# Aakash1312/Fluid-Simulation

Measured on AMD Instinct MI355X. Metric: simulated substeps/sec, higher is better.
Workload: dtype f64

## Files before the change

fluid-simulation_amd/csrc/common.h:

```cpp
#pragma once
#include <hip/hip_runtime.h>
#include <stdint.h>

namespace fl {

constexpr uint8_t F_SOLID = 1;
constexpr uint8_t F_FLUID = 2;
constexpr int F_CNT_SHIFT = 2;

struct Grid {
    int N;
    int lo;
    int hi;
    int nx, ny, nz;
    int ox, oy, oz;
    __host__ __device__ inline size_t idx(int ix, int iy, int iz) const
    {
        return ((size_t)ix * ny + (size_t)iy) * nz + (size_t)iz;
    }
    __host__ __device__ inline size_t cells() const { return (size_t)nx * ny * nz; }
    __host__ __device__ inline long sx() const { return (long)ny * nz; }
    __host__ __device__ inline int cx0() const { return lo + ox; }
    __host__ __device__ inline int cy0() const { return lo + oy; }
    __host__ __device__ inline int cz0() const { return lo + oz; }
    __host__ __device__ inline int cx1() const { return lo + ox + nx - 1; }
    __host__ __device__ inline int cy1() const { return lo + oy + ny - 1; }
    __host__ __device__ inline int cz1() const { return lo + oz + nz - 1; }
};

struct Box {
    int x0, y0, z0, x1, y1, z1;
    __host__ __device__ inline int nx() const { return x1 - x0 + 1; }
    __host__ __device__ inline int ny() const { return y1 - y0 + 1; }
    __host__ __device__ inline int nz() const { return z1 - z0 + 1; }
    __host__ __device__ inline long long cells() const { return (long long)nx() * ny() * nz(); }
};

template <typename T>
struct Coef {
    T diag[7];
    T inv[7];
    T off;
};

constexpr int LBOX_K0 = 16;
struct LBox {
    int x0, y0, z0, nx, ny, nz, Lx, Ly, Lz;
    __host__ __device__ inline size_t cells() const { return (size_t)Lx * Ly * Lz; }
};

struct MLevel {
    int dx, dy, dz;
    long sx, sy;
    int ox, oy, oz;
    size_t cells;
    __host__ __device__ inline size_t at(int i, int j, int k) const
    {
        return (size_t)((long)(i + ox) * sx + (long)(j + oy) * sy + (k + oz));
    }
};
template <typename T>
struct MgCoef {
    T diag[7];
    T inv[7];
    T off;
};

struct PcgState {
    double bb;
    double thr;
    double rr;
    int done;
    int iters;
    int breakdown;
    int pad;
};

struct StepState {
    int bbox_min[3];
    int bbox_max[3];
    int num_active;
    int n_out;
    int max_cell;
    int n_drop;
    int n_tl_mg, n_tl_sq;
    int n_rows, n_l1_old;
    int n_tl_int, n_tl_bnd;
    int n_l1_gal, n_drop_fail;
    unsigned long long max_speed_bits;
    double dt;
    double err_num;
    double err_den;
};

constexpr size_t STATE_PS_OFF = 256;
constexpr int MAX_PARTIALS = 8192;

__device__ __forceinline__ double spline(double x)
{
    if (x < 0) x *= -1.0;
    if (x < 0.5) return 1.5 * (4.0 * x * x * x - 4.0 * x * x + 2.0 / 3.0);
    if (x < 1.0) return 1.5 * ((-8.0 * (x * x * x) / 6.0) + 4.0 * x * x - 4.0 * x + 4.0 / 3.0);
    return 0;
}

__device__ __forceinline__ double spline_at(double p, int c, int d)
{
    double x = p - (double)c;
    if (d == 1) return spline(x);
    if (x < 0) x *= -1.0;
    if (x < 1.0) return 1.5 * ((-8.0 * (x * x * x) / 6.0) + 4.0 * x * x - 4.0 * x + 4.0 / 3.0);
    return 0;
}

template <typename T>
__device__ __forceinline__ T wave_sum(T v)
{
#pragma unroll
    for (int o = 32; o > 0; o >>= 1) v += __shfl_down(v, o, 64);
    return v;
}
template <typename T>
__device__ __forceinline__ T wave_max(T v)
{
#pragma unroll
    for (int o = 32; o > 0; o >>= 1) {
        T w = __shfl_down(v, o, 64);
        v = w > v ? w : v;
    }
    return v;
}
template <typename T, int NW>
__device__ __forceinline__ T block_sum(T v, T* sm)
{
    v = wave_sum(v);
    const int lane = threadIdx.x & 63, w = threadIdx.x >> 6;
    __syncthreads();
    if (lane == 0) sm[w] = v;
    __syncthreads();
    T r = 0;
    if (threadIdx.x == 0) {
#pragma unroll
        for (int i = 0; i < NW; ++i) r += sm[i];
    }
    return r;
}
template <int NW>
__device__ __forceinline__ double block_sum_array(const double* __restrict__ a, int n, double* sm)
{
    double v = 0;
    for (int i = threadIdx.x; i < n; i += NW * 64) v += a[i];
    v = wave_sum(v);
    const int lane = threadIdx.x & 63, w = threadIdx.x >> 6;
    __syncthreads();
    if (lane == 0) sm[w] = v;
    __syncthreads();
    if (threadIdx.x == 0) {
        double r = 0;
#pragma unroll
        for (int i = 0; i < NW; ++i) r += sm[i];
        sm[NW] = r;
    }
    __syncthreads();
    return sm[NW];
// ... 136 lines not shown
void launch_pcg_sq_list(hipStream_t st, LBox L, const uint8_t* cnt, const T* r, const T* s_in, T* s_out, T* q, Coef<T> cf,
                        const double* part_rr, int n_prev, const double* part_rz_new, const double* part_rz_old, double* part_pq, PcgState* ps,
                        int first, double tol, int n_rz, int zmode, const int* tlist, int nlist);
template <typename T>
void launch_pcg_xr_list(hipStream_t st, LBox L, const uint8_t* cnt, T* x, T* r, const T* s, const T* q, Coef<T> cf, const double* part_rz_cur,
                        int n_rz, const double* part_pq, double* part_rr, double* part_rz_next, PcgState* ps, const int* tlist, int nlist);
int pcg_row_count(const LBox& L);
int pcg_rows_blocks(int nrows);
void launch_row_list(hipStream_t st, LBox L, const uint8_t* cnt, int* flags, int* pos, int* list, int* block_sums, int* count);
constexpr int DROP_CAP = 65536;
constexpr int DROP_NCTR = 64;
void launch_drop_find(hipStream_t st, LBox L, uint8_t* cnt, int* ctr, int* pre, int* total, int* comp_n, int* comp_cells, const Box* own = nullptr);
void launch_drop_solve(hipStream_t st, Grid g, LBox L, int n_comp, const int* pre, const int* comp_n, const int* comp_cells, const uint8_t* flags,
                       const float* b, Coef<double> cf, double tol, double* pressure, double* keep, int* n_fail = nullptr, const PcgState* gate = nullptr);
template <typename T>
void launch_pcg_xr_rows(hipStream_t st, LBox L, const uint8_t* cnt, T* x, T* r, const T* s, const T* q, Coef<T> cf, const double* part_rz_cur,
                        int n_rz, const double* part_pq, int n_pq, double* part_rr, double* part_rz_next, PcgState* ps, const int* rlist, int nrows);
template <typename T>
void launch_pcg_sq_dist(hipStream_t st, LBox L, const uint8_t* cnt, const T* r, const T* s_in, T* s_out, T* q, Coef<T> cf, const double* g_rr,
                        const double* g_rz_new, const double* g_rz_old, double* part_pq, PcgState* ps, int first, double tol, int zmode);
template <typename T>
void launch_pcg_xr_dist(hipStream_t st, LBox L, const uint8_t* cnt, T* x, T* r, const T* s, const T* q, Coef<T> cf, const double* g_rz_cur,
                        const double* g_pq, double* part_rr, double* part_rz_next, PcgState* ps);
void launch_sum2(hipStream_t st, const double* a, int na, const double* b, int nb, double* out_a, double* out_b);
void launch_pcg_az_dist_zf(hipStream_t st, LBox L, const uint8_t* cnt, const float* z, double* w, Coef<double> cf, double* part_zw, PcgState* ps, const int* tlist, int nlist);
void launch_pcg_cgear_upd_zf(hipStream_t st, LBox L, const uint8_t* cnt, double* x, double* r, double* s, double* q, const float* z, const double* w, const double* g,
                             double* cg, int cur, double* part_rr, PcgState* ps, int first, double tol);
void launch_pcg_poll_stage(hipStream_t st, const double* part_rr, int n, const PcgState* ps, double* out);
void launch_pcg_poll_test(hipStream_t st, const double* g, PcgState* ps);
void launch_sum4(hipStream_t st, const double* a, int na, const double* b, int nb, const double* c, int nc, const double* e, int ne, double* out);
template <typename T>
void launch_pcg_az_dist(hipStream_t st, LBox L, const uint8_t* cnt, const T* z, T* w, Coef<T> cf, double* part_zw, PcgState* ps, const int* tlist = nullptr,
                        int nlist = 0);
template <typename T>
void launch_pcg_cgear_upd(hipStream_t st, LBox L, const uint8_t* cnt, T* x, T* r, T* s, T* q, const T* z, const T* w, const double* g, double* cg, int cur,
                          double* part_rr, PcgState* ps, int first, double tol);
template <typename T>
void launch_stencil_apply(hipStream_t st, Grid g, Box box, const uint8_t* flags, const T* s, T* q, Coef<T> cf);
template <typename T>
bool launch_stencil_march(hipStream_t st, Grid g, const uint8_t* flags, const T* s, T* q, Coef<T> cf, int variant, int cxcode);
template <typename T>
void launch_store_pressure(hipStream_t st, Grid g, LBox L, const uint8_t* cnt, const T* x, double* pressure, double* keep = nullptr,
                           const PcgState* ps = nullptr, bool gated = false);
template <typename T>
void launch_pcg_init_guess(hipStream_t st, Grid g, LBox L, const uint8_t* cnt, const float* b, const double* guess, const double* guess2, double ca,
                           double cb, T* x, T* r, Coef<T> cf, double* part_bb, double* part_rr0, PcgState* ps);

MLevel mg_level0(const LBox& L);
MLevel mg_coarser(const MLevel& f);
void launch_mg_type0(hipStream_t st, Grid g, LBox L, MLevel m, const uint8_t* flags, const uint8_t* cnt, uint8_t* typ);
void launch_mg_coarsen(hipStream_t st, MLevel mf, const uint8_t* tf, MLevel mc, uint8_t* tc, uint8_t* cnt_c);
void launch_mg_coarsen_types(hipStream_t st, MLevel mf, const uint8_t* tf, MLevel mc, uint8_t* tc);
void launch_mg_counts(hipStream_t st, MLevel m, const uint8_t* typ, uint8_t* cnt);
template <typename T>
void launch_mg_restrict(hipStream_t st, MLevel mf, const T* rf, MLevel mc, const uint8_t* cnt_c, T* fc, const PcgState* ps);
constexpr int MG_TAIL_MAX = 4;
constexpr size_t MG_TAIL_LDS = 144 * 1024;
size_t mg_tail_lds_bytes(int nl, const MLevel* lv, size_t elem);
int mg_up_blocks(const MLevel& m);
template <typename T, typename F>
void launch_mg_down(hipStream_t st, MLevel m, const uint8_t* cnt, const F* f, T* u, T* r, MLevel mc, const uint8_t* cnt_c, T* fc, MgCoef<T> cf,
                    const PcgState* ps, const int* tlist = nullptr, int nlist = 0, bool pcr = false);
template <typename T, typename F, typename O>
void launch_mg_up(hipStream_t st, MLevel m, const uint8_t* cnt, const F* f, const T* u, O* out, MLevel mc, const T* ec, MgCoef<T> cf,
                  double* part_dot, const PcgState* ps, double wc, const int* tlist = nullptr, int nlist = 0, const uint8_t* own = nullptr,
                  int pconst = 0);
bool gal_fits_coarsest(const MLevel& m);
void launch_gal_level1(hipStream_t st, MLevel m0, const uint8_t* cnt0, MgCoef<float> cf0, MLevel m1, float* gd, float* gx, float* gy, float* gz, uint8_t* cnt1);
void launch_gal_coarsen(hipStream_t st, MLevel mf, const float* fd, const float* fx, const float* fy, const float* fz, const uint8_t* cntf, MLevel mc,
                        float* gd, float* gx, float* gy, float* gz, uint8_t* cntc);
int gal_tile_count(const MLevel& m);
void launch_gal_tile_flags(hipStream_t st, MLevel m, const uint8_t* cnt, uint8_t* flags);
void launch_gal_down(hipStream_t st, MLevel m, const uint8_t* cnt, const float* gd, const float* gx, const float* gy, const float* gz, const float* f, float* u,
                     MLevel mc, float* fc, const PcgState* ps);
void launch_gal_up(hipStream_t st, MLevel m, const uint8_t* cnt, const float* gd, const float* gx, const float* gy, const float* gz, const float* f, const float* u,
                   float* out, MLevel mc, const float* ec, float wc, const PcgState* ps);
void launch_gal_coarsest(hipStream_t st, MLevel m, const float* gd, const float* gx, const float* gy, const float* gz, const float* f, float* u, int sweeps,
                         const PcgState* ps);
void launch_mg_tile_flags(hipStream_t st, MLevel m, const uint8_t* cnt, uint8_t* flags);
void launch_sq_tile_flags(hipStream_t st, LBox L, const uint8_t* cnt, uint8_t* flags);
int sq_tile_count(const LBox& L);
void launch_compact_flags(hipStream_t st, const uint8_t* flags, int n, int* list, int* count);
template <typename T>
void launch_mg_tail(hipStream_t st, int nl, const T* f0, const MLevel* lv, uint8_t* const* cnt, T* u0, const T* off, int sweeps, const PcgState* ps,
                    double wc);

}
```

fluid-simulation_amd/csrc/fluid_api.hip:

```cpp
#include "sim.h"
#include <algorithm>

using namespace fl;

static thread_local std::string g_err;
int fluid_fail(int code, const std::string& msg)
{
    g_err = msg;
    return code;
}
#define fail fluid_fail

Box fl::clip_dilate(const Box& b, int d, const Grid& g)
{
    Box r;
    r.x0 = b.x0 - d < 0 ? 0 : b.x0 - d;
    r.y0 = b.y0 - d < 0 ? 0 : b.y0 - d;
    r.z0 = b.z0 - d < 0 ? 0 : b.z0 - d;
    r.x1 = b.x1 + d > g.nx - 1 ? g.nx - 1 : b.x1 + d;
    r.y1 = b.y1 + d > g.ny - 1 ? g.ny - 1 : b.y1 + d;
    r.z1 = b.z1 + d > g.nz - 1 ? g.nz - 1 : b.z1 + d;
    return r;
}

// ... 151 lines not shown
    if (s->h_ss) hipHostFree(s->h_ss);
    if (s->h_small) hipHostFree(s->h_small);
    if (s->st) hipStreamDestroy(s->st);
    delete s;
    return FLUID_OK;
}

int fluid_create(const fluid_params_t* p, fluid_sim_t** out)
{
    if (!p || !out) return fail(FLUID_ERR_ARG, "null argument");
    Grid g;
    g.N = p->n;
    g.lo = -(p->n / 2);
    g.hi = g.lo + p->n - 1;
    g.nx = g.ny = g.nz = p->n;
    g.ox = g.oy = g.oz = 0;
    return fluid_create_window(p, g, out);
}

}

int fl::fluid_create_window(const fluid_params_t* p, const Grid& g, fluid_sim_t** out)
{
    if (!p || !out) return fail(FLUID_ERR_ARG, "null argument");
    if (p->n < 8 || p->n > 1024) return fail(FLUID_ERR_ARG, "n must be in [8,1024]");
    if (!(p->dx > 0) || !(p->rho > 0) || !(p->max_dt > 0)) return fail(FLUID_ERR_ARG, "dx, rho, max_dt must be > 0");
    if (p->precision != FLUID_PRECISION_FP64 && p->precision != FLUID_PRECISION_FP32) return fail(FLUID_ERR_ARG, "bad precision");
    if (!(p->flip_blend >= 0.0 && p->flip_blend <= 1.0)) return fail(FLUID_ERR_ARG, "flip_blend must be in [0,1] (1 = the reference's pure FLIP)");
    if (p->preconditioner != FLUID_PRECOND_MG && p->preconditioner != FLUID_PRECOND_JACOBI) return fail(FLUID_ERR_ARG, "bad preconditioner");
    if (p->solve_start != FLUID_START_WARM && p->solve_start != FLUID_START_ZERO) return fail(FLUID_ERR_ARG, "bad solve_start");
    if (p->mg_precision != FLUID_MG_FP32 && p->mg_precision != FLUID_MG_FP64) return fail(FLUID_ERR_ARG, "bad mg_precision");
    if (p->dist_solve < FLUID_DIST_AUTO || p->dist_solve > FLUID_DIST_REPLICATED || p->pad_ != 0) return fail(FLUID_ERR_ARG, "bad dist_solve / pad_");
    int ndev = 0;
    if (hipGetDeviceCount(&ndev) != hipSuccess || ndev <= 0)
        return fail(FLUID_ERR_HIP, "no HIP device visible: libfluid_hip has no CPU path");
    if (p->device < 0 || p->device >= ndev) return fail(FLUID_ERR_ARG, "device ordinal out of range");
    HIPCHK(hipSetDevice(p->device));
    fluid_sim* s = new fluid_sim();
    s->prm = *p;
    s->g = g;
    s->ncell = g.cells();
    s->dt = p->max_dt;
    s->mg_fp32 = p->mg_precision == FLUID_MG_FP32;
    s->warm = p->solve_start == FLUID_START_WARM;
    if (const char* e = getenv("FLUID_MG_CSWEEPS")) s->mg_csweeps = atoi(e);
    if (const char* e = getenv("FLUID_TILE_LISTS")) s->lists_force = atoi(e) != 0;
    if (const char* e = getenv("FLUID_P2G_FORM")) s->p2g_force = !strcmp(e, "rows") ? 1 : (!strcmp(e, "tiles") ? 2 : (!strcmp(e, "crowd") ? 3 : 0));
    if (const char* e = getenv("FLUID_MG_GALERKIN")) s->gal_mode = atoi(e);
    if (const char* e = getenv("FLUID_DROPLETS")) s->drops_on = atoi(e) != 0;
    if (const char* e = getenv("FLUID_ROW_SWEEPS")) s->row_sweeps = atoi(e) != 0;
    if (const char* e = getenv("FLUID_DROPLETS_MIN")) s->drop_min = atoi(e);
    if (const char* e = getenv("FLUID_ADVECT_BIN")) s->advect_bin = atoi(e) != 0;
    if (const char* e = getenv("FLUID_SOLVE_TAIL")) s->solve_tail = atoi(e) != 0;
    *out = nullptr;
    auto bail = [&](int rc) { fluid_destroy(s); return rc; };
#define A(expr) do { hipError_t e_ = (expr); if (e_ != hipSuccess) return bail(fail(FLUID_ERR_HIP, std::string(#expr) + ": " + hipGetErrorString(e_))); } while (0)
    A(hipStreamCreateWithFlags(&s->st, hipStreamNonBlocking));
    const size_t n = s->ncell;
    A(dalloc(&s->solid, n)); A(dalloc(&s->flags, n));
    A(dalloc(&s->container, n)); A(dalloc(&s->rhs, n)); A(dalloc(&s->diver, n)); A(dalloc(&s->diver2, n));
    A(dalloc(&s->u, n)); A(dalloc(&s->v, n)); A(dalloc(&s->w, n));
    A(dalloc(&s->ub, n)); A(dalloc(&s->vb, n)); A(dalloc(&s->wb, n));
    A(dalloc(&s->dcx, n)); A(dalloc(&s->dcy, n)); A(dalloc(&s->dcz, n));
    A(dalloc(&s->pressure, n));
    if (s->warm) {
        A(dalloc(&s->p_guess, n)); A(dalloc(&s->p_guess2, n));
        if (hipMemset(s->p_guess, 0, n * sizeof(double)) != hipSuccess || hipMemset(s->p_guess2, 0, n * sizeof(double)) != hipSuccess) return bail(FLUID_ERR_HIP);
        if (const char* e = getenv("FLUID_EXTRAPOLATE")) s->extrapolate = atoi(e) != 0;
        if (s->extrapolate) { A(dalloc(&s->p_q, n)); if (hipMemset(s->p_q, 0, n * sizeof(double)) != hipSuccess) return bail(FLUID_ERR_HIP); }
    }
    A(dalloc(&s->indices, n));
    A(dalloc(&s->scan_sums, (n + 2) / 2048 + 16));
    A(dalloc(&s->ipart, (size_t)1024 * 8));
    const size_t se = solver_elem(s);
    s->lmax = lbox_max_cells(std::max(g.nx, std::max(g.ny, g.nz)));
    const size_t ln = s->lmax;
    A(dalloc((char**)&s->R, ln * se)); A(dalloc((char**)&s->S[0], 2 * ln * se + 256));
    s->S[1] = (char*)s->S[0] + ln * se;
    A(dalloc((char**)&s->Q, ln * se)); A(dalloc((char**)&s->X, ln * se)); A(dalloc(&s->cntL, ln + 64));
    A(dalloc(&s->mg_part, ln / 256 + 64));
    A(dalloc(&s->part_bb, (size_t)MAX_PARTIALS)); A(dalloc(&s->part_rr, (size_t)MAX_PARTIALS));
    A(dalloc(&s->part_rz[0], (size_t)MAX_PARTIALS)); A(dalloc(&s->part_rz[1], (size_t)MAX_PARTIALS));
    A(dalloc(&s->part_pq, (size_t)MAX_PARTIALS)); A(dalloc(&s->part_err, (size_t)2 * MAX_PARTIALS));
    static_assert(sizeof(StepState) <= STATE_PS_OFF, "PcgState overlaps StepState");
    A(dalloc((char**)&s->ss, STATE_PS_OFF + sizeof(PcgState)));
    s->ps = (PcgState*)((char*)s->ss + STATE_PS_OFF);
    A(dalloc(&s->cell_count, n + 4)); A(dalloc(&s->cell_start, n + 4));
    A(dalloc(&s->d_small, (size_t)32));
    A(hipHostMalloc((void**)&s->h_small, 32 * sizeof(int)));
    A(hipEventCreateWithFlags(&s->ev_poll[0], hipEventDisableTiming));
    A(hipEventCreateWithFlags(&s->ev_poll[1], hipEventDisableTiming));
    A(hipHostMalloc((void**)&s->h_ss, STATE_PS_OFF + 2 * sizeof(PcgState)));
    s->h_ps = (PcgState*)((char*)s->h_ss + STATE_PS_OFF);
#undef A
    std::vector<uint8_t> sol(n, 0);
    const int N = p->n;
    for (int x = 0; x < g.nx; ++x)
        for (int y = 0; y < g.ny; ++y)
            for (int z = 0; z < g.nz; ++z) {
                const int X = x + g.ox, Y = y + g.oy, Z = z + g.oz;
                if (X < 2 || X > N - 3 || Y < 2 || Y > N - 3 || Z < 2 || Z > N - 3) sol[g.idx(x, y, z)] = 1;
            }
    hipError_t e = hipMemcpy(s->solid, sol.data(), n, hipMemcpyHostToDevice);
    if (e == hipSuccess) e = hipMemcpy(s->flags, sol.data(), n, hipMemcpyHostToDevice);
    if (e == hipSuccess) e = hipDeviceSynchronize();
    if (e != hipSuccess) return bail(fail(FLUID_ERR_HIP, std::string("solid upload: ") + hipGetErrorString(e)));
// ... 263 lines not shown
    int rc = phase_sort(s);
    if (rc) return rc;
    rc = clear_dirty(s);
    if (rc) return rc;
    memset(&s->stats, 0, sizeof(s->stats));
    s->stats.dt_in = s->dt;
    s->stats.dt_out = s->dt;
    for (int a = 0; a < 3; ++a) {
        s->stats.box_lo[a] = (&s->Rb.x0)[a];
        s->stats.box_hi[a] = (&s->Rb.x1)[a];
    }
    if (!box_empty(s->Rb)) {
        int tok = prof_begin(s, FLUID_PROF_P2G, (double)s->Rb.cells());
        rc = run_p2g(s, s->Rb);
        prof_end(s, FLUID_PROF_P2G, tok);
        if (rc) return rc;
        HIPCHK(hipGetLastError());
        s->dirty = s->Sb;
    }
    s->have_p2g = true;
    s->step_counter++;
    s->have_flags = false;
    return FLUID_OK;
}

template <typename T>
Coef<T> fl::make_coef(const fluid_sim* s)
{
    const double scale = s->dt / (s->prm.rho * s->prm.dx * s->prm.dx);
    Coef<T> c;
    float acc = 0.0f;
    c.diag[0] = 0;
    c.inv[0] = 0;
    for (int k = 1; k <= 6; ++k) {
        acc = (float)((double)acc + scale);
        c.diag[k] = (T)acc;
        c.inv[k] = (T)1 / c.diag[k];
    }
    c.off = (T)(float)(-1 * scale);
    return c;
}
template Coef<double> fl::make_coef<double>(const fluid_sim*);
template Coef<float> fl::make_coef<float>(const fluid_sim*);

hipError_t fl::zero_search(fluid_sim* s, size_t lb)
{
    const size_t step = (lb + 255) / 256 * 256;
    s->S[1] = (char*)s->S[0] + step;
    return hipMemsetAsync(s->S[0], 0, step + lb, s->st);
}


static int gal_build(fluid_sim* s);
static int mg_setup(fluid_sim* s)
{
    s->mgl[0] = mg_level0(s->L);
    int nl = 1;
    while (nl < fluid_sim::MG_MAXL && (nl < 2 || s->mgl[nl - 1].dx > 8 || s->mgl[nl - 1].dy > 8 || s->mgl[nl - 1].dz > 8)) {
        s->mgl[nl] = mg_coarser(s->mgl[nl - 1]);
        ++nl;
    }
    if (s->mgl[nl - 1].dx > 8 || s->mgl[nl - 1].dy > 8 || s->mgl[nl - 1].dz > 8) return fail(FLUID_ERR_STATE, "multigrid: too many levels");
    s->mg_nl = nl;
    int tail = nl - 1;
    const size_t es = s->mg_fp32 ? sizeof(float) : sizeof(double);
    auto fits = [&](int t) {
        const size_t b = nl - t <= MG_TAIL_MAX ? mg_tail_lds_bytes(nl - t, s->mgl + t, es) : 0;
        return b > 0 && b <= MG_TAIL_LDS;
    };
    while (tail > 1 && fits(tail - 1)) --tail;
    if (!fits(tail)) return fail(FLUID_ERR_STATE, "multigrid: coarsest level does not fit the tail kernel");
    s->mg_tail = tail;
    size_t total = 0;
    auto take = [&](size_t bytes) { const size_t o = total; total += (bytes + 255) / 256 * 256; return o; };
    size_t o_typ[fluid_sim::MG_MAXL], o_cnt[fluid_sim::MG_MAXL], o_u[fluid_sim::MG_MAXL], o_v[fluid_sim::MG_MAXL], o_f[fluid_sim::MG_MAXL],
        o_r[fluid_sim::MG_MAXL];
    for (int l = 0; l < nl; ++l) {
        const size_t c = s->mgl[l].cells + 64;
        o_typ[l] = take(c); o_cnt[l] = take(c);
        o_u[l] = take(c * es); o_v[l] = take(c * es); o_f[l] = take(c * es); o_r[l] = take(c * es);
    }
    const size_t o_z = take((s->mgl[0].cells + 64) * 8);
    if (total > s->mg_slab_cap) {
        if (s->mg_slab) { HIPCHK(hipStreamSynchronize(s->st)); hipFree(s->mg_slab); s->mg_slab = nullptr; }
        const size_t cap = total + total / 4;
        HIPCHK(hipMalloc((void**)&s->mg_slab, cap));
        s->mg_slab_cap = cap;
    }
    for (int l = 0; l < nl; ++l) {
        s->mg_typ[l] = (uint8_t*)(s->mg_slab + o_typ[l]);
        s->mg_cnt[l] = l ? (uint8_t*)(s->mg_slab + o_cnt[l]) : nullptr;
        s->mg_u[l] = s->mg_slab + o_u[l]; s->mg_v[l] = s->mg_slab + o_v[l];
        s->mg_f[l] = l ? s->mg_slab + o_f[l] : nullptr;
        s->mg_r[l] = s->mg_slab + o_r[l];
    }
    s->Zmg = s->mg_slab + o_z;
    HIPCHK(hipMemsetAsync(s->mg_slab, 0, total, s->st));
    launch_mg_type0(s->st, s->g, s->L, s->mgl[0], s->flags, s->cntL, s->mg_typ[0]);
    for (int l = 1; l < nl; ++l) launch_mg_coarsen(s->st, s->mgl[l - 1], s->mg_typ[l - 1], s->mgl[l], s->mg_typ[l], s->mg_cnt[l]);
    { int rcg = gal_build(s); if (rcg) return rcg; }
    HIPCHK(hipGetLastError());
    return FLUID_OK;
}

MgCoef<double> fl::mg_coef(const fluid_sim* s, int level)
{
    MgCoef<double> c;
    if (level == 0) {
        const Coef<double> f = make_coef<double>(s);
        for (int k = 0; k < 7; ++k) { c.diag[k] = f.diag[k]; c.inv[k] = f.inv[k]; }
        c.off = f.off;
        return c;
    }
    const double scale = s->dt / (s->prm.rho * s->prm.dx * s->prm.dx) / std::pow(4.0, level);
    c.off = -scale;
    c.diag[0] = 0; c.inv[0] = 0;
    for (int k = 1; k < 7; ++k) { c.diag[k] = scale * k; c.inv[k] = 1.0 / c.diag[k]; }
    return c;
}

static int mg_rz_blocks(const fluid_sim* s) { return s->lists_on ? s->n_tl_mg : mg_up_blocks(s->mgl[0]); }

template <typename V>
static MgCoef<V> mg_coef_as(const fluid_sim* s, int level)
{
    const MgCoef<double> d = mg_coef(s, level);
    MgCoef<V> c;
    for (int k = 0; k < 7; ++k) { c.diag[k] = (V)d.diag[k]; c.inv[k] = (V)d.inv[k]; }
    c.off = (V)d.off;
    return c;
}
static int gal_build(fluid_sim* s)
{
    s->gal = false;
    s->gal_eligible = false;
    const int nl = s->mg_nl;
    int lc = 1;
    while (lc < nl - 1 && !gal_fits_coarsest(s->mgl[lc])) ++lc;
    if (!(s->gal_mode && s->lists_on && s->mg_fp32 && !s->dist && (long)s->mgl[0].dx * s->mgl[0].dy * s->mgl[0].dz > 200000 &&
          gal_fits_coarsest(s->mgl[lc]) && lc >= 2)) {
        s->gal_it[0] = s->gal_it[1] = -1;
        return FLUID_OK;
    }
    s->gal_eligible = true;
    bool use = s->gal_mode >= 2;
    if (s->gal_mode == 1) {
        if (s->gal_it[0] < 0) use = false;
        else if (s->gal_it[1] < 0) use = true;
        else {
            use = 21 * s->gal_it[1] < 20 * s->gal_it[0];
            if (++s->gal_since_probe >= 32) { use = !use; s->gal_since_probe = 0; }
        }
// ... 875 lines not shown
```

fluid-simulation_amd/csrc/kernels_mg.hip:

```cpp
#include "common.h"
#include <cstdlib>
#include <cstring>

namespace fl {

constexpr double MG_W1 = 0.5617, MG_W2 = 1.3895;

template <typename T>
__device__ __forceinline__ void mg_load_coef(T* sd, T* si, const MgCoef<T>& cf)
{
    if (threadIdx.x == 0) {
#pragma unroll
        for (int i = 0; i < 7; ++i) {
            sd[i] = cf.diag[i];
            si[i] = cf.inv[i];
        }
    }
    __syncthreads();
}

__device__ __forceinline__ bool mg_cell(const MLevel& m, long t, int& i, int& j, int& k)
{
    const unsigned n = (unsigned)m.dx * (unsigned)m.dy * (unsigned)m.dz;
    if (t >= (long)n) return false;
    const unsigned u = (unsigned)t, dz = (unsigned)m.dz, dy = (unsigned)m.dy;
    const unsigned q = u / dz;
    k = (int)(u - q * dz);
    const unsigned p = q / dy;
    j = (int)(q - p * dy);
    i = (int)p;
    return true;
}

__global__ __launch_bounds__(256) void k_mg_type0(Grid g, LBox L, MLevel m, const uint8_t* __restrict__ flags, const uint8_t* __restrict__ cnt,
                                                  uint8_t* __restrict__ typ)
{
    int i, j, k;
    if (!mg_cell(m, (long)blockIdx.x * 256 + threadIdx.x, i, j, k)) return;
    const int gx = L.x0 + i - 1, gy = L.y0 + j - 1, gz = L.z0 + k - 1;
    uint8_t t = 0;
    const size_t c = m.at(i, j, k);
    if (gx >= 0 && gx < g.nx && gy >= 0 && gy < g.ny && gz >= 0 && gz < g.nz) {
        const uint8_t f = flags[g.idx(gx, gy, gz)];
        t = (f & F_SOLID) ? 0 : (cnt[c] ? 2 : 1);
    }
    typ[c] = t;
}

__global__ __launch_bounds__(256) void k_mg_coarsen(MLevel mf, const uint8_t* __restrict__ tf, MLevel mc, uint8_t* __restrict__ tc)
{
    int I, J, K;
    if (!mg_cell(mc, (long)blockIdx.x * 256 + threadIdx.x, I, J, K)) return;
    bool any_air = false, all_solid = true;
#pragma unroll
    for (int a = 0; a < 8; ++a) {
        const int i = 2 * I + (a & 1), j = 2 * J + ((a >> 1) & 1), k = 2 * K + (a >> 2);
        uint8_t t = 0;
        if (i < mf.dx && j < mf.dy && k < mf.dz) t = tf[mf.at(i, j, k)];
        any_air |= (t == 1);
        all_solid &= (t == 0);
    }
    tc[mc.at(I, J, K)] = any_air ? 1 : (all_solid ? 0 : 2);
}

__global__ __launch_bounds__(256) void k_mg_cnt(MLevel m, const uint8_t* __restrict__ typ, uint8_t* __restrict__ cnt)
{
    int i, j, k;
    if (!mg_cell(m, (long)blockIdx.x * 256 + threadIdx.x, i, j, k)) return;
    const size_t c = m.at(i, j, k);
    uint8_t n = 0;
    if (typ[c] == 2) {
        n = (typ[c - m.sx] != 0) + (typ[c + m.sx] != 0) + (typ[c - m.sy] != 0) + (typ[c + m.sy] != 0) + (typ[c - 1] != 0) + (typ[c + 1] != 0);
    }
    cnt[c] = n;
}


struct IoPlain {
    template <typename X> static __device__ __forceinline__ X ld(const X* p) { return *p; }
    template <typename X> static __device__ __forceinline__ void st(X* p, X v) { *p = v; }
};
struct IoSc1 {
    template <typename X> static __device__ __forceinline__ X ld(const X* p) { return __hip_atomic_load(p, __ATOMIC_RELAXED, __HIP_MEMORY_SCOPE_AGENT); }
    template <typename X> static __device__ __forceinline__ void st(X* p, X v) { __hip_atomic_store(p, v, __ATOMIC_RELAXED, __HIP_MEMORY_SCOPE_AGENT); }
};


template <typename T, typename IO = IoPlain>
__device__ __forceinline__ void d_restrict(const MLevel& mf, const T* __restrict__ rf, const MLevel& mc, const uint8_t* __restrict__ cnt_c,
                                           T* __restrict__ fc, long t)
{
    int I, J, K;
    if (!mg_cell(mc, t, I, J, K)) return;
    const size_t C = mc.at(I, J, K);
    T out = 0;
    if (!cnt_c[C]) return;
    {
        auto w = [](int a) { return (a == 0 || a == 3) ? (T)0.25 : (T)0.75; };
        const int i0 = 2 * I - 1, j0 = 2 * J - 1, k0 = 2 * K - 1;
        T acc = 0;
        if (i0 >= 0 && i0 + 3 < mf.dx && j0 >= 0 && j0 + 3 < mf.dy && k0 >= 0 && k0 + 3 < mf.dz) {
            const T* p = rf + mf.at(i0, j0, k0);
#pragma unroll
            for (int a = 0; a < 4; ++a) {
#pragma unroll
                for (int b = 0; b < 4; ++b) {
                    const T* q = p + a * mf.sx + b * mf.sy;
                    acc += w(a) * w(b) * ((T)0.25 * (q[0] + q[3]) + (T)0.75 * (q[1] + q[2]));
                }
            }
        } else {
            for (int a = 0; a < 4; ++a) {
                const int i = i0 + a;
                if (i < 0 || i >= mf.dx) continue;
                for (int b = 0; b < 4; ++b) {
                    const int j = j0 + b;
                    if (j < 0 || j >= mf.dy) continue;
                    T row = 0;
#pragma unroll
                    for (int d = 0; d < 4; ++d) {
                        const int k = k0 + d;
// ... 583 lines not shown
#undef TV
#undef TF
#undef TC
}

template <typename T>
__global__ __launch_bounds__(1024) void k_mg_tail(MgTail<T> a, const PcgState* ps)
{
    extern __shared__ double tail_lds[];
    __shared__ T sd[MG_TAIL_MAX][8], si[MG_TAIL_MAX][8];
    if (ps && ps->done) return;
    mg_tail_body<T, IoPlain>(a, tail_lds, sd, si, threadIdx.x);
}

static inline unsigned mg_blocks(const MLevel& m) { return (unsigned)(((long)m.dx * m.dy * m.dz + 255) / 256); }

MLevel mg_level0(const LBox& L)
{
    MLevel m;
    m.dx = L.nx + 2; m.dy = L.ny + 2; m.dz = L.nz + 2;
    m.sx = (long)L.Ly * L.Lz; m.sy = L.Lz;
    m.ox = 0; m.oy = 0; m.oz = LBOX_K0 - 1;
    m.cells = L.cells() + 2 * (size_t)L.Lz;
    return m;
}
MLevel mg_coarser(const MLevel& f)
{
    MLevel m;
    m.dx = (f.dx + 1) / 2; m.dy = (f.dy + 1) / 2; m.dz = (f.dz + 1) / 2;
    const int Lz = (16 + m.dz + 1 + 15) / 16 * 16;
    m.sy = Lz; m.sx = (long)(m.dy + 2) * Lz;
    m.ox = 1; m.oy = 1; m.oz = 16;
    m.cells = (size_t)(m.dx + 2) * m.sx + Lz;
    return m;
}

void launch_mg_type0(hipStream_t st, Grid g, LBox L, MLevel m, const uint8_t* flags, const uint8_t* cnt, uint8_t* typ)
{
    hipLaunchKernelGGL(k_mg_type0, dim3(mg_blocks(m)), dim3(256), 0, st, g, L, m, flags, cnt, typ);
}
void launch_mg_coarsen_types(hipStream_t st, MLevel mf, const uint8_t* tf, MLevel mc, uint8_t* tc)
{
    if (mg_blocks(mc)) hipLaunchKernelGGL(k_mg_coarsen, dim3(mg_blocks(mc)), dim3(256), 0, st, mf, tf, mc, tc);
}
void launch_mg_counts(hipStream_t st, MLevel m, const uint8_t* typ, uint8_t* cnt)
{
    if (mg_blocks(m)) hipLaunchKernelGGL(k_mg_cnt, dim3(mg_blocks(m)), dim3(256), 0, st, m, typ, cnt);
}
void launch_mg_coarsen(hipStream_t st, MLevel mf, const uint8_t* tf, MLevel mc, uint8_t* tc, uint8_t* cnt_c)
{
    hipLaunchKernelGGL(k_mg_coarsen, dim3(mg_blocks(mc)), dim3(256), 0, st, mf, tf, mc, tc);
    hipLaunchKernelGGL(k_mg_cnt, dim3(mg_blocks(mc)), dim3(256), 0, st, mc, (const uint8_t*)tc, cnt_c);
}
template <typename T>
void launch_mg_restrict(hipStream_t st, MLevel mf, const T* rf, MLevel mc, const uint8_t* cnt_c, T* fc, const PcgState* ps)
{
    if (mg_blocks(mc)) hipLaunchKernelGGL((k_mg_restrict<T>), dim3(mg_blocks(mc)), dim3(256), 0, st, mf, rf, mc, cnt_c, fc, ps);
}
constexpr int MG_TX = 8, MG_TY = 8, MG_TZ = 16;
constexpr int MG_RX = 8, MG_RY = 8, MG_RZ = 8;
constexpr unsigned MG_FEW_TILES = 384;
template <int TX, int TY, int TZ>
__global__ __launch_bounds__(256) void k_mg_tile_flags(MLevel m, const uint8_t* __restrict__ cnt, int gx, int gy, uint8_t* __restrict__ flags)
{
    const int tile = blockIdx.x;
    const int tbx = tile % gx, tby = (tile / gx) % gy, tbz = tile / (gx * gy);
    const int i0 = tbz * TX, j0 = tby * TY, k0 = tbx * TZ;
    int any = 0;
    for (int t = threadIdx.x; t < TX * TY * TZ; t += 256) {
        const int z = t % TZ, y = (t / TZ) % TY, x = t / (TZ * TY);
        const int i = i0 + x, j = j0 + y, k = k0 + z;
        if (i < m.dx && j < m.dy && k < m.dz) any |= cnt[m.at(i, j, k)];
    }
    any = __syncthreads_or(any);
    if (threadIdx.x == 0) flags[tile] = any != 0;
}

static inline bool mg_ng4() { return true; }
static inline dim3 mg_tiles(const MLevel& m, int tx, int ty, int tz)
{
    return dim3((unsigned)((m.dz + tz - 1) / tz), (unsigned)((m.dy + ty - 1) / ty), (unsigned)((m.dx + tx - 1) / tx));
}
int mg_up_blocks(const MLevel& m)
{
    const dim3 g = mg_tiles(m, MG_TX, MG_TY, MG_TZ);
    return (int)(g.x * g.y * g.z);
}
template <typename T, typename F>
void launch_mg_down(hipStream_t st, MLevel m, const uint8_t* cnt, const F* f, T* u, T* r, MLevel mc, const uint8_t* cnt_c, T* fc, MgCoef<T> cf,
                    const PcgState* ps, const int* tlist, int nlist, bool pcr)
{
    if (m.dx <= 0 || m.dy <= 0 || m.dz <= 0) return;
    if (fc && !pcr) {
        const dim3 g = mg_tiles(m, MG_RX, MG_RY, MG_RZ);
        if (sizeof(F) == sizeof(T) && g.x * g.y * g.z <= MG_FEW_TILES && mg_ng4())
            hipLaunchKernelGGL((k_mg_down<T, F, MG_RX, MG_RY, MG_RZ, true, 4>), dim3(g.x * g.y * g.z), dim3(1024), 0, st, m, cnt, f, u, r, mc, cnt_c, fc, cf,
                               ps, (int)g.x, (int)g.y, (const int*)nullptr);
        else
            hipLaunchKernelGGL((k_mg_down<T, F, MG_RX, MG_RY, MG_RZ, true>), dim3(g.x * g.y * g.z), dim3(256), 0, st, m, cnt, f, u, r, mc, cnt_c, fc, cf,
                               ps, (int)g.x, (int)g.y, (const int*)nullptr);
    } else {
        const dim3 g = mg_tiles(m, MG_TX, MG_TY, MG_TZ);
        hipLaunchKernelGGL((k_mg_down<T, F, MG_TX, MG_TY, MG_TZ, false>), dim3(tlist ? (unsigned)nlist : g.x * g.y * g.z), dim3(256), 0, st, m, cnt, f, u,
                           r, mc, cnt_c, fc, cf, ps, (int)g.x, (int)g.y, tlist);
    }
}
// ... 90 lines not shown
```

fluid-simulation_amd/csrc/sim.h:

```cpp
#pragma once
#include "common.h"
#include "../../include/fluid_hip.h"

#include <cmath>
#include <cstdio>
#include <cstdlib>
#include <cstring>
#include <string>
#include <utility>
#include <vector>

int fluid_fail(int code, const std::string& msg);
#define HIPCHK(expr)                                                                                              \
    do {                                                                                                          \
        hipError_t e_ = (expr);                                                                                   \
        if (e_ != hipSuccess)                                                                                     \
            return fluid_fail(FLUID_ERR_HIP, std::string(#expr) + ": " + hipGetErrorString(e_) + " @" + std::to_string(__LINE__)); \
    } while (0)

using namespace fl;

struct ProfClass {
    long launches = 0, sampled = 0;
    double ms = 0, cells = 0;
// ... 56 lines not shown
    double* pw = nullptr;
    double* p2g_part = nullptr;
    size_t p2g_part_cap = 0;
    int2* p2g_crowd = nullptr;
    size_t p2g_crowd_cap = 0;
    int* p2g_items = nullptr;
    size_t p2g_items_cap = 0;
    int max_cell = 0;
    uint8_t* tl_flags = nullptr;
    int *tl_mg = nullptr, *tl_sq = nullptr;
    size_t tl_cap = 0;
    int n_tl_mg = 0, n_tl_sq = 0;
    int *row_flags = nullptr, *row_pos = nullptr, *row_list = nullptr;
    size_t row_cap = 0;
    int n_rows = 0;
    bool rows_on = true;
    bool drops_on = true;
    bool row_sweeps = true;
    int* drop_ctr = nullptr;
    int* drop_n = nullptr;
    int* drop_cells = nullptr;
    int n_drop = 0;
    int drop_last = -1;
    int drop_min = 4000;
    int drop_skipped = 0;
    bool lists_hint = false;
    bool lists_on = false;
    int lists_force = -1;
    int p2g_force = 0;
    long p2g_ref_cells = 0;
    long last_num_active = 0;
    StepState* ss = nullptr;
    StepState* h_ss = nullptr;
    Box Pb{0, 0, 0, -1, -1, -1}, Rb{0, 0, 0, -1, -1, -1}, Sb{0, 0, 0, -1, -1, -1};
    Box dirty{0, 0, 0, -1, -1, -1};
    int flag_x0 = 0, flag_x1 = -1;
    bool flags_valid = false;
    bool sorted = false, have_p2g = false, have_flags = false;
    long n_out = 0;
    bool sort_hint = false;
    bool advect_bin = true;
    bool binned = false;
    int bin_x0 = 0, bin_x1 = -1;
    int bin_min[3] = {0, 0, 0}, bin_max[3] = {-1, -1, -1}, bin_n_out = 0, bin_max_cell = 0;
    bool solve_tail = true;
    bool tail_ran = false;
    double dt = 0.1;
    fluid_step_stats_t stats{};
    static constexpr int MG_MAXL = 8;
    int mg_nl = 0, mg_tail = 0;
    long mg_last_iters_k[3] = {0, 0, 0};
    int pass_class() const { return stats.outer_passes < 2 ? stats.outer_passes : 2; }
    int mg_csweeps = 3;
    MLevel mgl[MG_MAXL];
    uint8_t *mg_typ[MG_MAXL] = {}, *mg_cnt[MG_MAXL] = {};
    int gal_mode = 1;
    int gal_it[2] = {-1, -1};
    int gal_since_probe = 0;
    bool gal_eligible = false;
    bool gal = false;
    int gal_lc = 0;
    double gal_dt = 0;
    double gal_wc = 1.8;
    int gal_sweeps = 3;
    char* gal_slab = nullptr;
    size_t gal_slab_cap = 0;
    float* gal_c[MG_MAXL][4] = {};
    uint8_t* gal_cnt[MG_MAXL] = {};
    uint8_t* gal_tfl[MG_MAXL] = {};
    char *mg_u[MG_MAXL] = {}, *mg_v[MG_MAXL] = {}, *mg_f[MG_MAXL] = {}, *mg_r[MG_MAXL] = {};
    double mg_wc[4] = {1.25, 1.1, 1.0, 1.0};
    bool mg_fp32 = true;
    double* mg_part = nullptr;
    char* mg_slab = nullptr;
    size_t mg_slab_cap = 0;
    bool dist = false;
    struct DistState* ds = nullptr;
    long p_off = 0;
    int* d_small = nullptr;
    int* h_small = nullptr;
    struct SrcSlot {
        bool on = false;
        fluid_source_t src{};
        Box box{};
        int* buf = nullptr;
    };
    SrcSlot src[FLUID_MAX_SOURCES];
    Box sink[FLUID_MAX_SINKS] = {};
    bool sink_on[FLUID_MAX_SINKS] = {};
    int* src_sums = nullptr;
    long n_steps = 0;
    bool vel_ok = false;
    long src_emit_last = 0, src_rm_last = 0, src_emit_total = 0, src_rm_total = 0;
    struct OutState* out = nullptr;
    int out_every = 0;
    int prof_every = 0;
    ProfClass prof[FLUID_PROF_COUNT];
};

namespace fl {
inline bool box_empty(const Box& b) { return b.x1 < b.x0 || b.y1 < b.y0 || b.z1 < b.z0; }
Box clip_dilate(const Box& b, int d, const Grid& g);
template <typename T>
inline hipError_t dalloc(T** p, size_t n)
{
    hipError_t e = hipMalloc((void**)p, n * sizeof(T));
// ... 37 lines not shown
```

Baseline: 155.6.

## Build multigrid type pyramid in fused brick kernel and use exact div6

Replaces the per-level type0/coarsen/count kernel chain with a brick-based kernel. It computes several coarsened type levels in shared memory, followed by one kernel for the remaining top levels and one batched count kernel for all levels. This cuts the kernel launches and global round trips in multigrid setup. The spline's division by six is also replaced by a reciprocal multiply with an FMA correction, meant to stay exact. The new path adds more code complexity and uses large shared-memory bricks.

```diff
diff --git a/fluid-simulation_amd/csrc/common.h b/fluid-simulation_amd/csrc/common.h
--- a/fluid-simulation_amd/csrc/common.h
+++ b/fluid-simulation_amd/csrc/common.h
@@ -1,6 +1,7 @@
 #pragma once
 #include <hip/hip_runtime.h>
 #include <stdint.h>
+#include "exact_div.h"
 
 namespace fl {
 
@@ -100,7 +101,7 @@
 {
     if (x < 0) x *= -1.0;
     if (x < 0.5) return 1.5 * (4.0 * x * x * x - 4.0 * x * x + 2.0 / 3.0);
-    if (x < 1.0) return 1.5 * ((-8.0 * (x * x * x) / 6.0) + 4.0 * x * x - 4.0 * x + 4.0 / 3.0);
+    if (x < 1.0) return 1.5 * ((div6(-8.0 * (x * x * x))) + 4.0 * x * x - 4.0 * x + 4.0 / 3.0);
     return 0;
 }
 
@@ -109,7 +110,7 @@
     double x = p - (double)c;
     if (d == 1) return spline(x);
     if (x < 0) x *= -1.0;
-    if (x < 1.0) return 1.5 * ((-8.0 * (x * x * x) / 6.0) + 4.0 * x * x - 4.0 * x + 4.0 / 3.0);
+    if (x < 1.0) return 1.5 * ((div6(-8.0 * (x * x * x))) + 4.0 * x * x - 4.0 * x + 4.0 / 3.0);
     return 0;
 }
 
@@ -352,6 +353,9 @@
 void launch_mg_coarsen(hipStream_t st, MLevel mf, const uint8_t* tf, MLevel mc, uint8_t* tc, uint8_t* cnt_c);
 void launch_mg_coarsen_types(hipStream_t st, MLevel mf, const uint8_t* tf, MLevel mc, uint8_t* tc);
 void launch_mg_counts(hipStream_t st, MLevel m, const uint8_t* typ, uint8_t* cnt);
+constexpr int MG_PYR_MAXL = 8;
+void launch_mg_build(hipStream_t st, Grid g, LBox L, int nl, const MLevel* lv, uint8_t* const* typ, uint8_t* const* cnt, const uint8_t* flags,
+                     const uint8_t* cnt0, int brick_levels);
 template <typename T>
 void launch_mg_restrict(hipStream_t st, MLevel mf, const T* rf, MLevel mc, const uint8_t* cnt_c, T* fc, const PcgState* ps);
 constexpr int MG_TAIL_MAX = 4;
diff --git a/fluid-simulation_amd/csrc/exact_div.h b/fluid-simulation_amd/csrc/exact_div.h
--- /dev/null
+++ b/fluid-simulation_amd/csrc/exact_div.h
@@ -0,0 +1,30 @@
+#pragma once
+#include <math.h>
+
+#if defined(__HIPCC__) || defined(__CUDACC__)
+#define FL_HD __host__ __device__
+#else
+#define FL_HD
+#endif
+
+#ifndef FLUID_EXACT_DIV6
+#define FLUID_EXACT_DIV6 1
+#endif
+
+namespace fl {
+
+FL_HD inline double div6(double a)
+{
+#if FLUID_EXACT_DIV6
+    const double C = 1.0 / 6.0;
+    const double q0 = a * C;
+    const double r = fma(-6.0, q0, a);
+    return fma(r, C, q0);
+#else
+    return a / 6.0;
+#endif
+}
+
+}
+
+#undef FL_HD
diff --git a/fluid-simulation_amd/csrc/fluid_api.hip b/fluid-simulation_amd/csrc/fluid_api.hip
--- a/fluid-simulation_amd/csrc/fluid_api.hip
+++ b/fluid-simulation_amd/csrc/fluid_api.hip
@@ -227,6 +227,7 @@
     if (const char* e = getenv("FLUID_DROPLETS_MIN")) s->drop_min = atoi(e);
     if (const char* e = getenv("FLUID_ADVECT_BIN")) s->advect_bin = atoi(e) != 0;
     if (const char* e = getenv("FLUID_SOLVE_TAIL")) s->solve_tail = atoi(e) != 0;
+    if (const char* e = getenv("FLUID_MG_BUILD")) s->mg_build = atoi(e);
     *out = nullptr;
     auto bail = [&](int rc) { fluid_destroy(s); return rc; };
 #define A(expr) do { hipError_t e_ = (expr); if (e_ != hipSuccess) return bail(fail(FLUID_ERR_HIP, std::string(#expr) + ": " + hipGetErrorString(e_))); } while (0)
@@ -596,6 +597,7 @@
 
 
 static int gal_build(fluid_sim* s);
+static_assert(fluid_sim::MG_MAXL <= MG_PYR_MAXL, "launch_mg_build holds every level");
 static int mg_setup(fluid_sim* s)
 {
     s->mgl[0] = mg_level0(s->L);
@@ -640,8 +642,12 @@
     }
     s->Zmg = s->mg_slab + o_z;
     HIPCHK(hipMemsetAsync(s->mg_slab, 0, total, s->st));
-    launch_mg_type0(s->st, s->g, s->L, s->mgl[0], s->flags, s->cntL, s->mg_typ[0]);
-    for (int l = 1; l < nl; ++l) launch_mg_coarsen(s->st, s->mgl[l - 1], s->mg_typ[l - 1], s->mgl[l], s->mg_typ[l], s->mg_cnt[l]);
+    if (s->mg_build) {
+        launch_mg_build(s->st, s->g, s->L, nl, s->mgl, s->mg_typ, s->mg_cnt, s->flags, s->cntL, s->mg_build == 2 ? 2 : 4);
+    } else {
+        launch_mg_type0(s->st, s->g, s->L, s->mgl[0], s->flags, s->cntL, s->mg_typ[0]);
+        for (int l = 1; l < nl; ++l) launch_mg_coarsen(s->st, s->mgl[l - 1], s->mg_typ[l - 1], s->mgl[l], s->mg_typ[l], s->mg_cnt[l]);
+    }
     { int rcg = gal_build(s); if (rcg) return rcg; }
     HIPCHK(hipGetLastError());
     return FLUID_OK;
diff --git a/fluid-simulation_amd/csrc/kernels_mg.hip b/fluid-simulation_amd/csrc/kernels_mg.hip
--- a/fluid-simulation_amd/csrc/kernels_mg.hip
+++ b/fluid-simulation_amd/csrc/kernels_mg.hip
@@ -67,6 +67,122 @@
 {
     int i, j, k;
     if (!mg_cell(m, (long)blockIdx.x * 256 + threadIdx.x, i, j, k)) return;
+    const size_t c = m.at(i, j, k);
+    uint8_t n = 0;
+    if (typ[c] == 2) {
+        n = (typ[c - m.sx] != 0) + (typ[c + m.sx] != 0) + (typ[c - m.sy] != 0) + (typ[c + m.sy] != 0) + (typ[c - 1] != 0) + (typ[c + 1] != 0);
+    }
+    cnt[c] = n;
+}
+
+struct MgPyr {
+    int nl;
+    MLevel m[MG_PYR_MAXL];
+    uint8_t* typ[MG_PYR_MAXL];
+    uint8_t* cnt[MG_PYR_MAXL];
+    unsigned cb[MG_PYR_MAXL + 1];
+    unsigned tb[MG_PYR_MAXL + 1];
+};
+__device__ __forceinline__ uint8_t mg_type_of(bool any_air, bool all_solid) { return any_air ? 1 : (all_solid ? 0 : 2); }
+
+template <int BL, int l>
+__device__ __forceinline__ void mg_pyr_level(const MgPyr& P, const uint8_t* sf, uint8_t* sc)
+{
+    constexpr int S = BL - l, B = 1 << S, F = 2 * B;
+    for (int t = threadIdx.x; t < B * B * B; t += 256) {
+        const int Z = t & (B - 1), Y = (t >> S) & (B - 1), X = t >> (2 * S);
+        bool any_air = false, all_solid = true;
+#pragma unroll
+        for (int a = 0; a < 8; ++a) {
+            const uint8_t v = sf[((2 * X + (a & 1)) * F + 2 * Y + ((a >> 1) & 1)) * F + 2 * Z + (a >> 2)];
+            any_air |= (v == 1);
+            all_solid &= (v == 0);
+        }
+        const uint8_t v = mg_type_of(any_air, all_solid);
+        sc[t] = v;
+        const int I = (int)blockIdx.z * B + X, J = (int)blockIdx.y * B + Y, K = (int)blockIdx.x * B + Z;
+        if (l < P.nl && I < P.m[l].dx && J < P.m[l].dy && K < P.m[l].dz) P.typ[l][P.m[l].at(I, J, K)] = v;
+    }
+    __syncthreads();
+    if constexpr (l < BL) mg_pyr_level<BL, l + 1>(P, sc, sc + B * B * B);
+}
+
+template <int BL>
+__global__ __launch_bounds__(256) void k_mg_types(Grid g, LBox L, MgPyr P, const uint8_t* __restrict__ flags, const uint8_t* __restrict__ cnt0)
+{
+    constexpr int B = 1 << BL, N = B * B * B;
+    __shared__ uint8_t sp[N + N / 8 + N / 64 + N / 512 + 8];
+    const MLevel& m = P.m[0];
+    uint8_t* __restrict__ typ = P.typ[0];
+    const int ib = (int)blockIdx.z * B, jb = (int)blockIdx.y * B, kb = (int)blockIdx.x * B;
+    constexpr int NT = N < 256 ? 1 : N / 256;
+#pragma unroll
+    for (int q = 0; q < NT; ++q) {
+        const int t = (int)threadIdx.x + 256 * q;
+        if (t < N) {
+            const int z = t & (B - 1), y = (t >> BL) & (B - 1), x = t >> (2 * BL);
+            const int i = ib + x, j = jb + y, k = kb + z;
+            uint8_t v = 0;
+            if (i < m.dx && j < m.dy && k < m.dz) {
+                const int gx = L.x0 + i - 1, gy = L.y0 + j - 1, gz = L.z0 + k - 1;
+                const size_t c = m.at(i, j, k);
+                if (gx >= 0 && gx < g.nx && gy >= 0 && gy < g.ny && gz >= 0 && gz < g.nz) {
+                    const uint8_t f = flags[g.idx(gx, gy, gz)];
+                    v = (f & F_SOLID) ? 0 : (cnt0[c] ? 2 : 1);
+                }
+                typ[c] = v;
+            }
+            sp[t] = v;
+        }
+    }
+    __syncthreads();
+    mg_pyr_level<BL, 1>(P, sp, sp + N);
+}
+
+__device__ __forceinline__ int mg_pyr_pick(const MgPyr& P, const unsigned* first, unsigned b, MLevel& m, uint8_t*& typ, uint8_t*& cnt, unsigned& b0)
+{
+    int l = 1;
+    m = P.m[1]; typ = P.typ[1]; cnt = P.cnt[1]; b0 = first[1];
+#pragma unroll
+    for (int q = 2; q < MG_PYR_MAXL; ++q) {
+        if (q < P.nl && b >= first[q]) { l = q; m = P.m[q]; typ = P.typ[q]; cnt = P.cnt[q]; b0 = first[q]; }
+    }
+    return l;
+}
+
+__global__ __launch_bounds__(256) void k_mg_types_top(MgPyr P, int lb)
+{
+    MLevel m, mb = P.m[1];
+    uint8_t *typ, *cnt;
+    const uint8_t* tb = P.typ[1];
+    unsigned b0;
+    const int l = mg_pyr_pick(P, P.tb, blockIdx.x, m, typ, cnt, b0);
+#pragma unroll
+    for (int q = 2; q < MG_PYR_MAXL; ++q)
+        if (q == lb) { mb = P.m[q]; tb = P.typ[q]; }
+    int I, J, K;
+    if (!mg_cell(m, (long)(blockIdx.x - b0) * 256 + threadIdx.x, I, J, K)) return;
+    const int sh = l - lb, w = 1 << sh;
+    const int i1 = min((I << sh) + w, mb.dx), j1 = min((J << sh) + w, mb.dy), k1 = min((K << sh) + w, mb.dz);
+    bool any_air = false, all_solid = true;
+    for (int i = I << sh; i < i1; ++i)
+        for (int j = J << sh; j < j1; ++j)
+            for (int k = K << sh; k < k1; ++k) {
+                const uint8_t v = tb[mb.at(i, j, k)];
+                any_air |= (v == 1);
+                all_solid &= (v == 0);
+            }
+    typ[m.at(I, J, K)] = mg_type_of(any_air, all_solid);
+}
+
+__global__ __launch_bounds__(256) void k_mg_cnt_all(MgPyr P)
+{
+    MLevel m;
+    uint8_t *typ, *cnt;
+    unsigned b0;
+    mg_pyr_pick(P, P.cb, blockIdx.x, m, typ, cnt, b0);
+    int i, j, k;
+    if (!mg_cell(m, (long)(blockIdx.x - b0) * 256 + threadIdx.x, i, j, k)) return;
     const size_t c = m.at(i, j, k);
     uint8_t n = 0;
     if (typ[c] == 2) {
@@ -756,6 +872,34 @@
     hipLaunchKernelGGL(k_mg_coarsen, dim3(mg_blocks(mc)), dim3(256), 0, st, mf, tf, mc, tc);
     hipLaunchKernelGGL(k_mg_cnt, dim3(mg_blocks(mc)), dim3(256), 0, st, mc, (const uint8_t*)tc, cnt_c);
 }
+template <int BL>
+static void launch_mg_types(hipStream_t st, Grid g, LBox L, const MgPyr& P, const uint8_t* flags, const uint8_t* cnt0)
+{
+    constexpr int B = 1 << BL;
+    const MLevel& m = P.m[0];
+    hipLaunchKernelGGL((k_mg_types<BL>), dim3((m.dz + B - 1) / B, (m.dy + B - 1) / B, (m.dx + B - 1) / B), dim3(256), 0, st, g, L, P, flags, cnt0);
+}
+void launch_mg_build(hipStream_t st, Grid g, LBox L, int nl, const MLevel* lv, uint8_t* const* typ, uint8_t* const* cnt, const uint8_t* flags,
+                     const uint8_t* cnt0, int brick_levels)
+{
+    MgPyr P{};
+    P.nl = nl;
+    for (int l = 0; l < MG_PYR_MAXL; ++l) {
+        const int q = l < nl ? l : nl - 1;
+        P.m[l] = lv[q]; P.typ[l] = typ[q]; P.cnt[l] = cnt[q];
+    }
+    const int BL = brick_levels == 2 ? 2 : 4;
+    unsigned nc = 0, nt = 0;
+    for (int l = 1; l <= MG_PYR_MAXL; ++l) {
+        P.cb[l] = nc; P.tb[l] = nt;
+        if (l < nl) nc += mg_blocks(lv[l]);
+        if (l < nl && l > BL) nt += mg_blocks(lv[l]);
+    }
+    if (BL == 2) launch_mg_types<2>(st, g, L, P, flags, cnt0);
+    else launch_mg_types<4>(st, g, L, P, flags, cnt0);
+    if (nt) hipLaunchKernelGGL(k_mg_types_top, dim3(nt), dim3(256), 0, st, P, BL);
+    if (nc) hipLaunchKernelGGL(k_mg_cnt_all, dim3(nc), dim3(256), 0, st, P);
+}
 template <typename T>
 void launch_mg_restrict(hipStream_t st, MLevel mf, const T* rf, MLevel mc, const uint8_t* cnt_c, T* fc, const PcgState* ps)
 {
diff --git a/fluid-simulation_amd/csrc/sim.h b/fluid-simulation_amd/csrc/sim.h
--- a/fluid-simulation_amd/csrc/sim.h
+++ b/fluid-simulation_amd/csrc/sim.h
@@ -132,6 +132,7 @@
     long mg_last_iters_k[3] = {0, 0, 0};
     int pass_class() const { return stats.outer_passes < 2 ? stats.outer_passes : 2; }
     int mg_csweeps = 3;
+    int mg_build = 1;
     MLevel mgl[MG_MAXL];
     uint8_t *mg_typ[MG_MAXL] = {}, *mg_cnt[MG_MAXL] = {};
     int gal_mode = 1;
```

New measurement: 155.5, median of 2. About the same (-0.0%).
